# zjykzj/YOLOv4

Hardware: AMD Instinct MI355X
Metric: images/sec fwd+bwd @608x608 bs=64 per GPU (YOLOv4 training step: forward + YOLOLoss + backward) (higher is better)
Workload: dtype f32

## Files before the change

yolov4_amd/csrc/common.h:

```cpp
#pragma once
#include <hip/hip_runtime.h>
#include <stdint.h>
#include "../../include/yolov4_amd.h"

typedef float f32x4 __attribute__((ext_vector_type(4)));
typedef float f32x16 __attribute__((ext_vector_type(16)));
typedef unsigned int u32x4 __attribute__((ext_vector_type(4)));

#define Y4_CHECK_LAUNCH()                                   \
    do {                                                    \
        if (hipGetLastError() != hipSuccess) return Y4_ERR_LAUNCH; \
    } while (0)

static inline hipStream_t y4_stream(void* s) { return reinterpret_cast<hipStream_t>(s); }

#include <atomic>
struct Y4DynLds {
    std::atomic<unsigned long long> done{0ull};
    bool ensure(const void* kernel, size_t bytes) {
        int d = 0;
        if (hipGetDevice(&d) != hipSuccess) return false;
        if (d >= 0 && d < 64 && ((done.load(std::memory_order_acquire) >> d) & 1ull)) return true;
        if (hipFuncSetAttribute(kernel, hipFuncAttributeMaxDynamicSharedMemorySize, (int)bytes) != hipSuccess) return false;
        if (d >= 0 && d < 64) done.fetch_or(1ull << d, std::memory_order_release);
        return true;
    }
};

__device__ __forceinline__ float y4_mish(float x) {
    const float n = __expf(fminf(x, 20.0f));
    const float w = n * (n + 2.0f);
    return x * (w * __frcp_rn(w + 2.0f));
}
__device__ __forceinline__ float y4_mish_grad(float x) {
    const float n = __expf(fminf(x, 20.0f));
    const float w = n * (n + 2.0f);
    const float rd = __frcp_rn(w + 2.0f);
    const float q = fmaf(n, n, n);
    return fmaf(4.0f * (x * q), rd, w) * rd;
}
__device__ __forceinline__ float y4_act(float x, int act) {
    switch (act) {
        case Y4_ACT_LEAKY: return x > 0.0f ? x : 0.1f * x;
        case Y4_ACT_MISH: return y4_mish(x);
        case Y4_ACT_RELU: return fmaxf(x, 0.0f);
        default: return x;
    }
}
__device__ __forceinline__ float y4_act_grad(float x, int act) {
    switch (act) {
        case Y4_ACT_LEAKY: return x > 0.0f ? 1.0f : 0.1f;
        case Y4_ACT_MISH: return y4_mish_grad(x);
        case Y4_ACT_RELU: return x > 0.0f ? 1.0f : 0.0f;
        default: return 1.0f;
    }
}

template <int ACT> __device__ __forceinline__ float y4_act_t(float x) {
// ... 26 lines not shown
```

yolov4_amd/csrc/conv_planes.hip:

```cpp
#include <stdlib.h>
#include <type_traits>
#include "common.h"
#include "conv_geom.h"

namespace {

typedef _Float16 f16x8 __attribute__((ext_vector_type(8)));
typedef float f32x4v __attribute__((ext_vector_type(4)));

__device__ __host__ __forceinline__ unsigned pl_scale_exp(unsigned amax_bits) {
    const unsigned e = (amax_bits >> 23) & 0xffu;
    if (e == 0u || e == 255u) return 127u;
    int se = 268 - (int)e;
    if (se < 2) se = 2;
    if (se > 252) se = 252;
    return (unsigned)se;
}
__device__ __forceinline__ float pl_scale(const unsigned* amax) { return __uint_as_float(pl_scale_exp(amax ? *amax : 0u) << 23); }
__device__ __forceinline__ float pl_unscale(const unsigned* amax) { return __uint_as_float((254u - pl_scale_exp(amax ? *amax : 0u)) << 23); }

struct PlaneConvGeom {
    const unsigned char* src;
    const unsigned char* wt;
    float* dst; long long ldd;
    const float* res; long long ldr;
    float* stats;
    int dst_bf16;
    int cls_ntaps, cls_ph, cls_pw, Hfull, Wfull;
    int cls_dh[4], cls_dw[4], cls_slot[4];
    int B, Hs, Ws, Cs, Hd, Wd, N, k, stride, pad, M, K;
    int mtiles, ntiles;
    unsigned long long src_total_bytes;
    unsigned wt_bytes;
    const unsigned* src_amax; const unsigned* wt_amax;
};

constexpr int PROW = 128;

typedef __bf16 bf16x8 __attribute__((ext_vector_type(8)));
template <bool BF>
__device__ __forceinline__ f32x4v pl_mma(const f16x8 a, const f16x8 b, const f32x4v c) {
    if constexpr (BF) return __builtin_amdgcn_mfma_f32_16x16x32_bf16(__builtin_bit_cast(bf16x8, a), __builtin_bit_cast(bf16x8, b), c, 0, 0, 0);
    else return __builtin_amdgcn_mfma_f32_16x16x32_f16(a, b, c, 0, 0, 0);
}

#ifndef PL_ST_POL
#define PL_ST_POL 2
#endif
template <int BM, int BN, int WM, int WN, bool BF, bool YB = false, bool DG2 = false>
__global__ __launch_bounds__(WM * WN * 64, WM * WN == 8 ? 1 : 2) void conv_planes_mfma(const PlaneConvGeom g) {
    constexpr int NWAVE = WM * WN, NTHR = NWAVE * 64;
    static_assert(NWAVE == 8 || NWAVE == 4, "8 or 4 waves");
    constexpr int WTM = BM / WM, WTN = BN / WN, TM = WTM / 16, TN = WTN / 16;
    constexpr int A_BYTES = BM * PROW, B_BYTES = BN * PROW, STAGE = A_BYTES + B_BYTES;
    constexpr int NSTAGE = (NWAVE == 8 && 3 * STAGE <= 160 * 1024) ? 3 : 2;
    constexpr int KSH = BF ? 6 : 5;
    constexpr unsigned WEB = BF ? 2u : 4u;
    constexpr int PA = BM / 8 / NWAVE, PB = BN / 8 / NWAVE, NDMA = PA + PB;
    static_assert(PA >= 1 && PB >= 1 && ((NSTAGE == 3 && NDMA == 6) || (NSTAGE == 2 && NDMA == 8)),
                  "the counted vmcnt below assumes 6 (three stages) or 8 (two stages) pieces per wave and K-tile");
    typedef float accv __attribute__((ext_vector_type(4)));
    extern __shared__ __attribute__((aligned(1024))) unsigned char smem[];

    const int tid = threadIdx.x, lane = tid & 63;
    const int wave = __builtin_amdgcn_readfirstlane(tid >> 6);
    const int wm = wave / WN, wn = wave % WN;
    const int lt = y4_xcd_remap(blockIdx.x, g.mtiles * g.ntiles);
    const int mt = lt / g.ntiles, nt = lt - mt * g.ntiles;
    const int n0 = nt * BN;
    const int CC = g.Cs >> KSH;
    const int KT = (DG2 ? g.cls_ntaps : g.k * g.k) * CC;

    const int pix_per_img = g.Hd * g.Wd;
    const int b_first = (int)(((long long)mt * BM) / pix_per_img);
    const unsigned pitch = (unsigned)g.Cs * 4u;
    const unsigned long long img_bytes = (unsigned long long)g.Hs * g.Ws * pitch;
    const unsigned long long skip = (unsigned long long)b_first * img_bytes;
    const unsigned long long left = g.src_total_bytes > skip ? g.src_total_bytes - skip : 0ull;
    const __amdgpu_buffer_rsrc_t src_rsrc = y4_make_rsrc(g.src + skip, (unsigned)(left < 0xfffffff0ull ? left : 0xfffffff0ull));
    const __amdgpu_buffer_rsrc_t wt_rsrc = y4_make_rsrc(g.wt, g.wt_bytes);
    const unsigned OOB = 0xffffffffu;

    const int lr = lane >> 3, pos = lane & 7;
    unsigned a_base[PA], a_valid[PA], a_voff[PA];
#pragma unroll
    for (int i = 0; i < PA; ++i) {
        const int row = (wave * PA + i) * 8 + lr;
        const int m = mt * BM + row;
        const bool ok = m < g.M;
        const int mm = ok ? m : 0;
        const int b = mm / pix_per_img;
        const int rem = mm - b * pix_per_img;
        const int hd = rem / g.Wd, wd = rem - hd * g.Wd;
        const int hc = DG2 ? hd : hd * g.stride - g.pad, wc = DG2 ? wd : wd * g.stride - g.pad;
        const int chunk = pos ^ ((row >> 1) & 7);
        a_base[i] = (unsigned)(((b - b_first) * g.Hs + hc) * g.Ws + wc) * pitch + (unsigned)chunk * 16u;
        unsigned v = 0u;
        if constexpr (DG2) {
            for (int t = 0; t < g.cls_ntaps; ++t)
                if (ok && hc + g.cls_dh[t] < g.Hs && wc + g.cls_dw[t] < g.Ws) v |= 1u << t;
        } else {
            for (int r = 0; r < g.k; ++r)
                for (int q = 0; q < g.k; ++q)
                    if (ok && (unsigned)(hc + r) < (unsigned)g.Hs && (unsigned)(wc + q) < (unsigned)g.Ws) v |= 1u << (r * g.k + q);
        }
        a_valid[i] = v;
    }
    unsigned b_off[PB];
#pragma unroll
    for (int j = 0; j < PB; ++j) {
        const int row = (wave * PB + j) * 8 + lr;
        const int chunk = pos ^ ((row >> 1) & 7);
        b_off[j] = (n0 + row) < g.N ? (unsigned)(n0 + row) * (unsigned)g.K * WEB + (unsigned)chunk * 16u : OOB;
    }
    int ld_tap = 0, ld_r = 0, ld_q = 0, ld_cc = 0;
    int ld_slot = DG2 ? g.cls_slot[0] : 0;
    auto tap_setup = [&]() {
        unsigned toff;
        if constexpr (DG2) {
            const int t = ld_tap < g.cls_ntaps ? ld_tap : 0;
            toff = (unsigned)(g.cls_dh[t] * g.Ws + g.cls_dw[t]) * pitch;
            ld_slot = g.cls_slot[t];
        } else {
            toff = (unsigned)(ld_r * g.Ws + ld_q) * pitch;
            ld_slot = ld_tap;
        }
#pragma unroll
        for (int i = 0; i < PA; ++i) a_voff[i] = ((a_valid[i] >> ld_tap) & 1u) ? a_base[i] + toff : OOB;
    };
    tap_setup();
    typedef __attribute__((address_space(3))) void* lds_ptr;
    auto issue = [&](int stage, auto P0, auto P1) {
        constexpr int p0 = decltype(P0)::value, p1 = decltype(P1)::value;
        unsigned char* st = smem + stage * STAGE;
        const unsigned soff_a = (unsigned)ld_cc * 128u;
        const unsigned soff_b = (unsigned)(ld_slot * CC + ld_cc) * 128u;
#pragma unroll
        for (int p = p0; p < p1; ++p) {
            if (p < PA)
                __builtin_amdgcn_raw_ptr_buffer_load_lds(src_rsrc, (lds_ptr)(st + (wave * PA + p) * 1024), 16, (int)a_voff[p], (int)soff_a, 0, 0);
            else
                __builtin_amdgcn_raw_ptr_buffer_load_lds(wt_rsrc, (lds_ptr)(st + A_BYTES + (wave * PB + (p - PA)) * 1024), 16,
                                                         (int)b_off[p - PA], (int)soff_b, 0, 0);
        }
        if constexpr (p1 == NDMA) {
            if (++ld_cc == CC) {
                ld_cc = 0; ++ld_tap;
                if (++ld_q == g.k) { ld_q = 0; ++ld_r; }
                tap_setup();
            }
        }
    };
    using I0 = std::integral_constant<int, 0>; using I2 = std::integral_constant<int, 2>; using I4 = std::integral_constant<int, 4>;
    using I6 = std::integral_constant<int, NDMA>;

    accv acc0[TM][TN], acc1[BF ? 1 : TM][BF ? 1 : TN];
#pragma unroll
    for (int i = 0; i < TM; ++i)
#pragma unroll
        for (int j = 0; j < TN; ++j)
#pragma unroll
            for (int e = 0; e < 4; ++e) {
                acc0[i][j][e] = 0.f;
                if constexpr (!BF) acc1[i][j][e] = 0.f;
            }

    const int fr = lane & 15, kq = lane >> 4;
    const int sw = (fr >> 1) & 7;
    const int a_hi = (wm * WTM + fr) * PROW + ((kq ^ sw) << 4), a_lo = (wm * WTM + fr) * PROW + (((4 + kq) ^ sw) << 4);
    const int b_hi = A_BYTES + (wn * WTN + fr) * PROW + ((kq ^ sw) << 4), b_lo = A_BYTES + (wn * WTN + fr) * PROW + (((4 + kq) ^ sw) << 4);

    bool pend = false;
    auto step = [&](auto SC, const int kt) {
        constexpr int S = decltype(SC)::value;
        const unsigned char* base = smem + S * STAGE;
        f16x8 fb[TN][2];
#pragma unroll
        for (int j = 0; j < TN; ++j) {
            fb[j][0] = *reinterpret_cast<const f16x8*>(base + b_hi + j * 16 * PROW);
            fb[j][1] = *reinterpret_cast<const f16x8*>(base + b_lo + j * 16 * PROW);
        }
        f16x8 fap[2][2];
        fap[0][0] = *reinterpret_cast<const f16x8*>(base + a_hi);
        fap[0][1] = *reinterpret_cast<const f16x8*>(base + a_lo);
#pragma unroll
        for (int i = 0; i < TM; ++i) {
            if (i + 1 < TM) {
                fap[(i + 1) & 1][0] = *reinterpret_cast<const f16x8*>(base + a_hi + (i + 1) * 16 * PROW);
                fap[(i + 1) & 1][1] = *reinterpret_cast<const f16x8*>(base + a_lo + (i + 1) * 16 * PROW);
            }
            const f16x8 fa0 = fap[i & 1][0], fa1 = fap[i & 1][1];
            if (i == TM - 1) {
                __builtin_amdgcn_sched_barrier(0);
                asm volatile("s_waitcnt lgkmcnt(0)" ::: "memory");
                if (kt + 1 < KT) {
                    if constexpr (NSTAGE == 3) {
                        if (kt + 2 < KT) asm volatile("s_waitcnt vmcnt(6)" ::: "memory");
                        else asm volatile("s_waitcnt vmcnt(0)" ::: "memory");
                        __builtin_amdgcn_s_barrier();
                        if (kt + 3 < KT) { issue(S, I0{}, I2{}); pend = true; }
                    } else {
                        asm volatile("s_waitcnt vmcnt(0)" ::: "memory");
                        __builtin_amdgcn_s_barrier();
                        if (kt + 2 < KT) issue(S, I0{}, I6{});
                    }
                }
            }
            if constexpr (BF) {
#pragma unroll
                for (int j = 0; j < TN; ++j) acc0[i][j] = pl_mma<true>(fa0, fb[j][0], acc0[i][j]);
#pragma unroll
                for (int j = 0; j < TN; ++j) acc0[i][j] = pl_mma<true>(fa1, fb[j][1], acc0[i][j]);
            } else {
#pragma unroll
                for (int j = 0; j < TN; ++j) {
                    acc1[i][j] = pl_mma<false>(fa1, fb[j][0], acc1[i][j]);
                    acc1[i][j] = pl_mma<false>(fa0, fb[j][1], acc1[i][j]);
                    acc0[i][j] = pl_mma<false>(fa0, fb[j][0], acc0[i][j]);
                }
            }
            if constexpr (NSTAGE == 3) {
                if (i == 0 && pend) issue((S + 2) % NSTAGE, I2{}, I4{});
                if (i == 1 && pend) { issue((S + 2) % NSTAGE, I4{}, I6{}); pend = false; }
            }
        }
    };
    static_assert(TM >= 3, "the DMA pieces are spread over the first three row tiles");

    for (int t = 0; t < NSTAGE && t < KT; ++t) issue(t, I0{}, I6{});
    if constexpr (NSTAGE == 3) {
        if (KT >= 3) asm volatile("s_waitcnt vmcnt(12)" ::: "memory");
        else if (KT == 2) asm volatile("s_waitcnt vmcnt(6)" ::: "memory");
        else asm volatile("s_waitcnt vmcnt(0)" ::: "memory");
    } else {
        if (KT >= 2) asm volatile("s_waitcnt vmcnt(8)" ::: "memory");
        else asm volatile("s_waitcnt vmcnt(0)" ::: "memory");
    }
    __builtin_amdgcn_s_barrier();
    if constexpr (NSTAGE == 3) {
        int kt = 0;
        for (; kt + 3 <= KT; kt += 3) {
            step(std::integral_constant<int, 0>{}, kt);
            step(std::integral_constant<int, 1>{}, kt + 1);
            step(std::integral_constant<int, 2>{}, kt + 2);
        }
        if (kt < KT) step(std::integral_constant<int, 0>{}, kt);
        if (kt + 1 < KT) step(std::integral_constant<int, 1>{}, kt + 1);
    } else {
        int kt = 0;
        for (; kt + 2 <= KT; kt += 2) {
            step(std::integral_constant<int, 0>{}, kt);
            step(std::integral_constant<int, 1>{}, kt + 1);
        }
        if (kt < KT) step(std::integral_constant<int, 0>{}, kt);
    }

    const float un = BF ? 1.0f : pl_unscale(g.src_amax) * pl_unscale(g.wt_amax);
    const float un1 = un * (1.0f / 2048.0f);
    auto result = [&](int i, int j, int e) -> float {
        if constexpr (BF) return acc0[i][j][e];
        else return acc0[i][j][e] * un + acc1[i][j][e] * un1;
    };
    {
        const unsigned drow = (unsigned)g.ldd * 4u, rrow = (unsigned)g.ldr * 4u;
        const long long row0 = (long long)mt * BM;
        const unsigned long long left = (unsigned long long)(g.M - row0);
        const unsigned long long dby = left * drow, rby = g.ldr ? left * rrow : (unsigned long long)g.N * 4ull;
        const __amdgpu_buffer_rsrc_t drs = y4_make_rsrc(reinterpret_cast<char*>(g.dst) + row0 * (long long)drow, (unsigned)(dby < 0xfffffff0ull ? dby : 0xfffffff0ull));
        const __amdgpu_buffer_rsrc_t rrs = y4_make_rsrc(g.res ? reinterpret_cast<const char*>(g.res) + row0 * (long long)rrow : nullptr,
                                                        g.res ? (unsigned)(rby < 0xfffffff0ull ? rby : 0xfffffff0ull) : 0u);
        int lane_e = lane;
        asm volatile("" : "+v"(lane_e));
        const int fr = lane_e & 15, kq = lane_e >> 4;
        const int colb = n0 + wn * WTN + fr;
        const bool allc = n0 + BN <= g.N;
        if constexpr (DG2) {
            const __amdgpu_buffer_rsrc_t xrs = y4_make_rsrc(g.dst, (unsigned)((unsigned long long)g.B * g.Hfull * g.Wfull * drow));
#pragma unroll
            for (int i = 0; i < TM; ++i) {
                const int m0 = mt * BM + wm * WTM + 16 * i + 4 * kq;
                int b = m0 / pix_per_img;
                const int rem = m0 - b * pix_per_img;
                int hc = rem / g.Wd, wc = rem - hc * g.Wd;
#pragma unroll
                for (int e = 0; e < 4; ++e) {
                    const bool rok = m0 + e < g.M;
                    const unsigned po = (unsigned)((b * g.Hfull + 2 * hc + g.cls_ph) * g.Wfull + 2 * wc + g.cls_pw) * drow + (unsigned)colb * 4u;
#pragma unroll
                    for (int j = 0; j < TN; ++j) {
                        const float v = result(i, j, e);
// ... 45 lines not shown
                        const bool cok = allc || colb + 16 * j < g.N;
                        __builtin_amdgcn_raw_buffer_store_b32(__builtin_bit_cast(unsigned, v), drs, (int)(cok ? dvo + 64u * j : 0xffffffffu), (int)(e * drow), PL_ST_POL);
                    }
            }
        }
        } else {
            float csum[TN], cssum[TN];
#pragma unroll
            for (int j = 0; j < TN; ++j) { csum[j] = 0.f; cssum[j] = 0.f; }
#pragma unroll
            for (int i = 0; i < TM; ++i) {
                const unsigned rl = (unsigned)(wm * WTM + 16 * i + 4 * kq);
                const unsigned dvo = rl * drow + (unsigned)colb * 2u;
#pragma unroll
                for (int e = 0; e < 4; ++e)
#pragma unroll
                    for (int j = 0; j < TN; ++j) {
                        const float v = result(i, j, e);
                        unsigned u = __builtin_bit_cast(unsigned, v);
                        u = (u + 0x7fffu + ((u >> 16) & 1u)) & 0xffff0000u;
                        const float vr = __builtin_bit_cast(float, u);
                        csum[j] += vr; cssum[j] += vr * vr;
                        const unsigned nb = (unsigned)__builtin_amdgcn_update_dpp(0, (int)u, 0xB1, 0xf, 0xf, true);
                        const bool cok = (allc || colb + 16 * j < g.N) && !(fr & 1);
                        __builtin_amdgcn_raw_buffer_store_b32((u >> 16) | nb, drs, (int)(cok ? dvo + 32u * j : 0xffffffffu), (int)(e * drow), PL_ST_POL);
                    }
                __builtin_amdgcn_sched_barrier(0);
            }
#pragma unroll
            for (int j = 0; j < TN; ++j) { acc0[0][j][0] = csum[j]; acc0[0][j][1] = cssum[j]; }
        }
    }
    if (g.stats) {
        __syncthreads();
        float* red = reinterpret_cast<float*>(smem);
#pragma unroll
        for (int j = 0; j < TN; ++j) {
            float cs = 0.f, css = 0.f;
            if constexpr (YB) {
                cs = acc0[0][j][0]; css = acc0[0][j][1];
            } else {
#pragma unroll
                for (int i = 0; i < TM; ++i)
#pragma unroll
                    for (int e = 0; e < 4; ++e) { const float v = acc0[i][j][e]; cs += v; css += v * v; }
            }
            cs += __shfl_xor(cs, 16, 64); css += __shfl_xor(css, 16, 64);
            cs += __shfl_xor(cs, 32, 64); css += __shfl_xor(css, 32, 64);
            if (kq == 0) {
                const int c = wn * WTN + j * 16 + fr;
                red[(wm * BN + c) * 2 + 0] = cs;
                red[(wm * BN + c) * 2 + 1] = css;
            }
        }
        __syncthreads();
        for (int c = tid; c < BN; c += NTHR) {
            float cs = 0.f, css = 0.f;
#pragma unroll
            for (int w = 0; w < WM; ++w) { cs += red[(w * BN + c) * 2]; css += red[(w * BN + c) * 2 + 1]; }
            const int n = n0 + c;
            if (n < g.N) {
                g.stats[((long long)mt * 2 + 0) * g.N + n] = cs;
                g.stats[((long long)mt * 2 + 1) * g.N + n] = css;
            }
        }
    }
}

struct PlaneWgradGeom {
    const unsigned char* x;
    const unsigned char* dy;
    float* out;
    int B, H, W, Cin, Cout, k, pad, M, J;
    int ldy_ch;
    int ntn, ntj, splits, steps_per_split;
    unsigned long long x_total_bytes, dy_total_bytes;
    const unsigned* x_amax; const unsigned* dy_amax;
};

typedef __fp16 trh4 __attribute__((__vector_size__(4 * sizeof(__fp16))));
__device__ __forceinline__ f16x8 tr_frag(const unsigned char* p) {
    typedef __attribute__((address_space(3))) trh4* lp;
    const trh4 a = __builtin_amdgcn_ds_read_tr16_b64_v4f16((lp)(p));
    const trh4 b = __builtin_amdgcn_ds_read_tr16_b64_v4f16((lp)(p + 4 * PROW));
    f16x8 r;
#pragma unroll
    for (int e = 0; e < 4; ++e) { r[e] = (_Float16)a[e]; r[4 + e] = (_Float16)b[e]; }
    return r;
}

template <int N> __device__ __forceinline__ void pl_wait_vm() {
    static_assert(N == 0 || N == 3 || N == 4 || N == 6 || N == 8 || N == 12, "add the literal");
    if constexpr (N == 0) asm volatile("s_waitcnt vmcnt(0)" ::: "memory");
    else if constexpr (N == 3) asm volatile("s_waitcnt vmcnt(3)" ::: "memory");
    else if constexpr (N == 4) asm volatile("s_waitcnt vmcnt(4)" ::: "memory");
    else if constexpr (N == 6) asm volatile("s_waitcnt vmcnt(6)" ::: "memory");
    else if constexpr (N == 8) asm volatile("s_waitcnt vmcnt(8)" ::: "memory");
    else asm volatile("s_waitcnt vmcnt(12)" ::: "memory");
}
// ... 448 lines not shown
        if (nt == 1) return launch_stream_bf16<4, 1, 4, YB>(g, st, nparts);
        if (nt == 2) return launch_stream_bf16<4, 2, 4, YB>(g, st, nparts);
        return launch_stream_bf16<4, 4, 4, YB>(g, st, nparts);
    }
    if (nt == 1) return launch_stream_bf16<8, 1, 4, YB>(g, st, nparts);
    if (nt == 2) return launch_stream_bf16<8, 2, 4, YB>(g, st, nparts);
    return launch_stream_bf16<8, 4, 4, YB>(g, st, nparts);
}

__global__ __launch_bounds__(256) void bf16_filter_kernel(const float* __restrict__ w, unsigned short* __restrict__ fwd,
                                                          unsigned short* __restrict__ tr, int Cout, int Cin, int kk, int mirror) {
    const long long n = (long long)Cout * kk * Cin;
    const long long i0 = blockIdx.x * (long long)blockDim.x + threadIdx.x, step = (long long)gridDim.x * blockDim.x;
    if (fwd)
        for (long long i = i0; i < n; i += step) fwd[i] = pl_bf16_bits(w[i]);
    if (tr)
        for (long long i = i0; i < n; i += step) {
            const int nn = (int)(i % Cout);
            const long long t = i / Cout;
            const int tp = (int)(t % kk);
            const int tap = mirror ? kk - 1 - tp : tp;
            const int c = (int)(t / kk);
            tr[i] = pl_bf16_bits(w[((long long)nn * kk + tap) * Cin + c]);
        }
}
int bf16_filter(const float* w, unsigned short* fwd, unsigned short* tr, int Cout, int Cin, int kk, bool mirror, hipStream_t st) {
    const long long n = (long long)Cout * kk * Cin;
    const int blocks = (int)((n + 255) / 256 > 2048 ? 2048 : (n + 255) / 256);
    hipLaunchKernelGGL(bf16_filter_kernel, dim3(blocks > 0 ? blocks : 1), dim3(256), 0, st, w, fwd, tr, Cout, Cin, kk, mirror ? 1 : 0);
    Y4_CHECK_LAUNCH();
    return Y4_OK;
}

template <int BM, int BN, int WM, int WN, bool BF, bool YB = false, bool DG2 = false>
int launch_conv_planes(const PlaneConvGeom& g0, hipStream_t st) {
    PlaneConvGeom g = g0;
    g.mtiles = (g.M + BM - 1) / BM;
    g.ntiles = (g.N + BN - 1) / BN;
    constexpr int NW = WM * WN;
    constexpr size_t stage = (size_t)(BM + BN) * PROW;
    constexpr size_t smem = ((NW == 8 && 3 * stage <= 160 * 1024) ? 3ull : 2ull) * stage;
    static_assert(NW == 8 || 2 * smem <= 160 * 1024, "two blocks per CU");
    static_assert(smem <= 160 * 1024, "LDS");
    auto kern = conv_planes_mfma<BM, BN, WM, WN, BF, YB, DG2>;
    static Y4DynLds lds_attr;
    if (!lds_attr.ensure(reinterpret_cast<const void*>(kern), smem)) return Y4_ERR_LAUNCH;
    y4::note_kernel("conv_planes_mfma<%d, %d, %d, %d, %s, %s, %s>", BM, BN, WM, WN, BF ? "true" : "false", YB ? "true" : "false",
                    DG2 ? "true" : "false");
    hipLaunchKernelGGL(kern, dim3(g.mtiles * g.ntiles), dim3(NW * 64), smem, st, g);
    Y4_CHECK_LAUNCH();
    return Y4_OK;
}

}

namespace y4 {

bool planes_conv_ok(int Cin, int Cout, int k, int stride) {
    return Cin > 0 && (Cin & 31) == 0 && Cout > 0 && (Cout & 3) == 0 && (k == 1 || k == 3) && (stride == 1 || stride == 2);
}

static bool conv_window_ok(int B, int Hs, int Ws, int Cs, int N, int k, int stride, bool bf) {
    const int pad = (k - 1) / 2;
    const long long Hd = (Hs + 2 * pad - k) / stride + 1, Wd = (Ws + 2 * pad - k) / stride + 1;
    if (Hd <= 0 || Wd <= 0 || (long long)B * Hd * Wd >= (1ll << 31)) return false;
    const unsigned long long img = (unsigned long long)Hs * Ws * (unsigned long long)Cs * 4ull;
    const unsigned long long wb = (unsigned long long)N * k * k * Cs * (bf ? 2ull : 4ull);
    const unsigned long long imgs_per_tile = 256ull / (unsigned long long)(Hd * Wd) + 2;
    return img * imgs_per_tile < 0xfffffff0ull && wb < 0xfffffff0ull;
}
static bool dgrad_s2_window_ok(int B, int H, int W, int Cin, int Cout, long long lddx) {
    if ((H & 1) || (W & 1)) return false;
    return conv_window_ok(B, H / 2, W / 2, Cout, Cin, 3, 1, false) &&
           (unsigned long long)B * H * W * (unsigned long long)lddx * 4ull < 0xfffffff0ull;
}
static bool wgrad_window_ok(int B, int H, int W, int Cin, int Cout, int k, int stride, bool bf) {
    const long long M = (long long)B * H * W;
    if (M >= (1ll << 31) - 65536) return false;
    if ((unsigned long long)Cout * k * k * Cin * 4ull >= 0xfffffff0ull) return false;
    int ntn, ntj, splits, sps;
    planes_wgrad_plan(B, H, W, Cin, Cout, k, &ntn, &ntj, &splits, &sps, planes_wgrad_tn(Cout, bf), bf);
    const int pad = (k - 1) / 2;
// ... 34 lines not shown
    g.wt_bytes = (unsigned)wb;
    g.src_amax = src_amax; g.wt_amax = wt_amax;
    static const int small_mode = getenv("Y4_PLANES_SMALL") ? atoi(getenv("Y4_PLANES_SMALL")) : 1;
    bool quant = false;
    {
        const long long nt = (N + 127) / 128;
        const long long b256 = (long long)((g.M + 255) / 256) * nt, b128 = (long long)((g.M + 127) / 128) * nt;
        const long long c256 = ((b256 + 255) / 256) * 2;
        const long long tail = b128 % 512;
        const long long c128 = (b128 / 512) * 2 + (tail == 0 ? 0 : (tail <= 256 ? 1 : 2));
        quant = (double)c128 * 1.08 < (double)c256;
    }
    const bool small = small_mode == 2 || (small_mode == 1 && (g.K <= 256 || quant)) || (small_mode == 4 && g.K <= 256);
    if (bf && stream_bf16_ok(g, dst_bf16)) {
        g.K = Cs;
        return dst_bf16 ? dispatch_stream_bf16<true>(g, st, nparts) : dispatch_stream_bf16<false>(g, st, nparts);
    }
    if (bf) {
        const char* bt = getenv("Y4_BF_TILE");
        const int bf_tile = bt ? atoi(bt) : 0;
        const long long mt = (g.M + 255) / 256;
        const long long r256 = (mt * ((N + 255) / 256) + 255) / 256, r128 = (mt * ((N + 127) / 128) + 255) / 256;
        const bool big = bf_tile == 2 || (bf_tile == 0 && N > 128 && (double)r256 * 2.0 <= (double)r128 * 1.25);
        if (small && !big) {
            if (nparts) *nparts = (g.M + 127) / 128;
            return dst_bf16 ? launch_conv_planes<128, 128, 2, 2, true, true>(g, st) : launch_conv_planes<128, 128, 2, 2, true>(g, st);
        }
        if (nparts) *nparts = (g.M + 255) / 256;
        if (dst_bf16) return big ? launch_conv_planes<256, 256, 2, 4, true, true>(g, st) : launch_conv_planes<256, 128, 4, 2, true, true>(g, st);
        return big ? launch_conv_planes<256, 256, 2, 4, true>(g, st) : launch_conv_planes<256, 128, 4, 2, true>(g, st);
    }
    if (dst_bf16) return Y4_ERR_SHAPE;
    if (nparts) *nparts = small ? (g.M + 127) / 128 : (g.M + 255) / 256;
    return small ? launch_conv_planes<128, 128, 2, 2, false>(g, st) : launch_conv_planes<256, 128, 4, 2, false>(g, st);
}

int planes_dgrad_s2(const void* dy, const unsigned* dy_amax, const void* wt_planes, const unsigned* wt_amax, float* dx, long long lddx,
                    int B, int H, int W, int Cin, int Cout, hipStream_t st, bool bf) {
    if ((H & 1) || (W & 1) || (Cout & 31) || (Cin & 3) || (bf && (Cout & 63))) return Y4_ERR_SHAPE;
    const int Ho = H / 2, Wo = W / 2;
    PlaneConvGeom g{};
    g.src = static_cast<const unsigned char*>(dy); g.wt = static_cast<const unsigned char*>(wt_planes);
    g.dst = dx; g.ldd = lddx;
    g.B = B; g.Hs = Ho; g.Ws = Wo; g.Cs = Cout; g.N = Cin; g.k = 3; g.stride = 1; g.pad = 0;
    g.Hd = Ho; g.Wd = Wo; g.Hfull = H; g.Wfull = W;
    if (B <= 0 || Ho <= 0 || Wo <= 0 || !dgrad_s2_window_ok(B, H, W, Cin, Cout, lddx)) return Y4_ERR_SHAPE;
    const long long M = (long long)B * Ho * Wo;
    g.M = (int)M; g.K = 9 * Cout;
    const unsigned long long img = (unsigned long long)Ho * Wo * (unsigned long long)Cout * 4ull;
    const unsigned long long wb = (unsigned long long)Cin * g.K * (bf ? 2ull : 4ull);
    g.src_total_bytes = (unsigned long long)B * img;
    g.wt_bytes = (unsigned)wb;
    g.src_amax = dy_amax; g.wt_amax = wt_amax;
    for (int c = 3; c >= 0; --c) {
        const int ph = c >> 1, pw = c & 1;
        g.cls_ph = ph; g.cls_pw = pw; g.cls_ntaps = 0;
        for (int r = 0; r < 3; ++r)
            for (int q = 0; q < 3; ++q) {
                if (((ph + 1 - r) & 1) || ((pw + 1 - q) & 1)) continue;
                const int t = g.cls_ntaps++;
                g.cls_dh[t] = (ph + 1 - r) / 2; g.cls_dw[t] = (pw + 1 - q) / 2; g.cls_slot[t] = r * 3 + q;
            }
        const int rc = bf ? launch_conv_planes<256, 128, 4, 2, true, false, true>(g, st)
                          : launch_conv_planes<256, 128, 4, 2, false, false, true>(g, st);
        if (rc != Y4_OK) return rc;
    }
    return Y4_OK;
// ... 247 lines not shown
```

Baseline: 449.8.

## Make f32 planes conv kernel persistent with cross-tile DMA prefetch

Adds a persistent variant of the f32 planes MFMA conv kernel. The grid is capped at resident blocks (CU count times blocks per CU), and each block loops over output tiles. Per-tile row and filter offset tables are built in LDS and double-buffered, so the global-load pipeline can run straight into the next tile's K loop without draining. The aim is to remove the pipeline fill and drain at each tile and the wave-quantization tail. In exchange it adds LDS table reads in tap setup, extra barriers, and more LDS use, which could lower occupancy or stall. It is on by default through an environment variable.

```diff
diff --git a/yolov4_amd/csrc/common.h b/yolov4_amd/csrc/common.h
--- a/yolov4_amd/csrc/common.h
+++ b/yolov4_amd/csrc/common.h
@@ -24,6 +24,20 @@
         if (hipFuncSetAttribute(kernel, hipFuncAttributeMaxDynamicSharedMemorySize, (int)bytes) != hipSuccess) return false;
         if (d >= 0 && d < 64) done.fetch_or(1ull << d, std::memory_order_release);
         return true;
+    }
+};
+
+struct Y4CuCount {
+    std::atomic<int> n[64];
+    Y4CuCount() { for (auto& v : n) v.store(0, std::memory_order_relaxed); }
+    int get() {
+        int d = 0;
+        if (hipGetDevice(&d) != hipSuccess) return -1;
+        if (d >= 0 && d < 64) { const int c = n[d].load(std::memory_order_acquire); if (c > 0) return c; }
+        int c = 0;
+        if (hipDeviceGetAttribute(&c, hipDeviceAttributeMultiprocessorCount, d) != hipSuccess || c <= 0) return -1;
+        if (d >= 0 && d < 64) n[d].store(c, std::memory_order_release);
+        return c;
     }
 };
 
diff --git a/yolov4_amd/csrc/conv_planes.hip b/yolov4_amd/csrc/conv_planes.hip
--- a/yolov4_amd/csrc/conv_planes.hip
+++ b/yolov4_amd/csrc/conv_planes.hip
@@ -47,13 +47,40 @@
 #ifndef PL_ST_POL
 #define PL_ST_POL 2
 #endif
-template <int BM, int BN, int WM, int WN, bool BF, bool YB = false, bool DG2 = false>
-__global__ __launch_bounds__(WM * WN * 64, WM * WN == 8 ? 1 : 2) void conv_planes_mfma(const PlaneConvGeom g) {
+
+typedef unsigned long long pl_u64;
+__device__ __forceinline__ unsigned pl_lds_addr(const unsigned char* p) {
+    return (unsigned)(__UINTPTR_TYPE__)(__attribute__((address_space(3))) const unsigned char*)p;
+}
+__device__ __forceinline__ void pl_lds_st64(unsigned addr, unsigned lo, unsigned hi) {
+    const pl_u64 v = (pl_u64)lo | ((pl_u64)hi << 32);
+    asm volatile("ds_write_b64 %0, %1" ::"v"(addr), "v"(v) : "memory");
+}
+__device__ __forceinline__ void pl_lds_st32(unsigned addr, unsigned v) { asm volatile("ds_write_b32 %0, %1" ::"v"(addr), "v"(v) : "memory"); }
+__device__ __forceinline__ void pl_lds_ld64x4(unsigned addr, pl_u64 (&e)[4]) {
+    asm volatile("ds_read_b64 %0, %4\n\tds_read_b64 %1, %4 offset:64\n\tds_read_b64 %2, %4 offset:128\n\tds_read_b64 %3, %4 offset:192\n\t"
+                 "s_waitcnt lgkmcnt(0)"
+                 : "=&v"(e[0]), "=&v"(e[1]), "=&v"(e[2]), "=&v"(e[3]) : "v"(addr) : "memory");
+}
+template <int N> __device__ __forceinline__ void pl_lds_ld_hdr_rows(unsigned haddr, unsigned raddr, pl_u64& h0, unsigned& h1, unsigned (&r)[N]) {
+    static_assert(N == 2 || N == 4, "filter pieces per wave");
+    if constexpr (N == 2)
+        asm volatile("ds_read_b64 %0, %4\n\tds_read_b32 %1, %4 offset:8\n\tds_read_b32 %2, %5\n\tds_read_b32 %3, %5 offset:32\n\t"
+                     "s_waitcnt lgkmcnt(0)"
+                     : "=&v"(h0), "=&v"(h1), "=&v"(r[0]), "=&v"(r[1]) : "v"(haddr), "v"(raddr) : "memory");
+    else
+        asm volatile("ds_read_b64 %0, %6\n\tds_read_b32 %1, %6 offset:8\n\tds_read_b32 %2, %7\n\tds_read_b32 %3, %7 offset:32\n\t"
+                     "ds_read_b32 %4, %7 offset:64\n\tds_read_b32 %5, %7 offset:96\n\ts_waitcnt lgkmcnt(0)"
+                     : "=&v"(h0), "=&v"(h1), "=&v"(r[0]), "=&v"(r[1]), "=&v"(r[2]), "=&v"(r[3]) : "v"(haddr), "v"(raddr) : "memory");
+}
+template <int BM, int BN, int WM, int WN, bool BF, bool YB, bool DG2, bool PERSIST>
+__device__ __forceinline__ void conv_planes_body(const PlaneConvGeom& g) {
     constexpr int NWAVE = WM * WN, NTHR = NWAVE * 64;
     static_assert(NWAVE == 8 || NWAVE == 4, "8 or 4 waves");
     constexpr int WTM = BM / WM, WTN = BN / WN, TM = WTM / 16, TN = WTN / 16;
     constexpr int A_BYTES = BM * PROW, B_BYTES = BN * PROW, STAGE = A_BYTES + B_BYTES;
     constexpr int NSTAGE = (NWAVE == 8 && 3 * STAGE <= 160 * 1024) ? 3 : 2;
+    constexpr int RED_BYTES = WM * BN * 2 * 4;
     constexpr int KSH = BF ? 6 : 5;
     constexpr unsigned WEB = BF ? 2u : 4u;
     constexpr int PA = BM / 8 / NWAVE, PB = BN / 8 / NWAVE, NDMA = PA + PB;
@@ -65,27 +92,27 @@
     const int tid = threadIdx.x, lane = tid & 63;
     const int wave = __builtin_amdgcn_readfirstlane(tid >> 6);
     const int wm = wave / WN, wn = wave % WN;
-    const int lt = y4_xcd_remap(blockIdx.x, g.mtiles * g.ntiles);
-    const int mt = lt / g.ntiles, nt = lt - mt * g.ntiles;
-    const int n0 = nt * BN;
+    const int ntot = g.mtiles * g.ntiles;
+    const int G = PERSIST ? (int)gridDim.x : ntot;
+    const int NTAP = DG2 ? g.cls_ntaps : g.k * g.k;
     const int CC = g.Cs >> KSH;
-    const int KT = (DG2 ? g.cls_ntaps : g.k * g.k) * CC;
+    const int KT = NTAP * CC;
 
     const int pix_per_img = g.Hd * g.Wd;
-    const int b_first = (int)(((long long)mt * BM) / pix_per_img);
     const unsigned pitch = (unsigned)g.Cs * 4u;
     const unsigned long long img_bytes = (unsigned long long)g.Hs * g.Ws * pitch;
-    const unsigned long long skip = (unsigned long long)b_first * img_bytes;
-    const unsigned long long left = g.src_total_bytes > skip ? g.src_total_bytes - skip : 0ull;
-    const __amdgpu_buffer_rsrc_t src_rsrc = y4_make_rsrc(g.src + skip, (unsigned)(left < 0xfffffff0ull ? left : 0xfffffff0ull));
     const __amdgpu_buffer_rsrc_t wt_rsrc = y4_make_rsrc(g.wt, g.wt_bytes);
     const unsigned OOB = 0xffffffffu;
 
-    const int lr = lane >> 3, pos = lane & 7;
-    unsigned a_base[PA], a_valid[PA], a_voff[PA];
-#pragma unroll
-    for (int i = 0; i < PA; ++i) {
-        const int row = (wave * PA + i) * 8 + lr;
+    auto tile_origin = [&](const int ltile, int& mt, int& n0, int& b_first, unsigned long long& skip, unsigned& bytes) __attribute__((always_inline)) {
+        const int lt = y4_xcd_remap(ltile, ntot);
+        mt = lt / g.ntiles; n0 = (lt - mt * g.ntiles) * BN;
+        b_first = (int)(((long long)mt * BM) / pix_per_img);
+        skip = (unsigned long long)b_first * img_bytes;
+        const unsigned long long left = g.src_total_bytes > skip ? g.src_total_bytes - skip : 0ull;
+        bytes = (unsigned)(left < 0xfffffff0ull ? left : 0xfffffff0ull);
+    };
+    auto row_state = [&](const int mt, const int b_first, const int row, unsigned& base, unsigned& valid) __attribute__((always_inline)) {
         const int m = mt * BM + row;
         const bool ok = m < g.M;
         const int mm = ok ? m : 0;
@@ -93,8 +120,7 @@
         const int rem = mm - b * pix_per_img;
         const int hd = rem / g.Wd, wd = rem - hd * g.Wd;
         const int hc = DG2 ? hd : hd * g.stride - g.pad, wc = DG2 ? wd : wd * g.stride - g.pad;
-        const int chunk = pos ^ ((row >> 1) & 7);
-        a_base[i] = (unsigned)(((b - b_first) * g.Hs + hc) * g.Ws + wc) * pitch + (unsigned)chunk * 16u;
+        base = (unsigned)(((b - b_first) * g.Hs + hc) * g.Ws + wc) * pitch;
         unsigned v = 0u;
         if constexpr (DG2) {
             for (int t = 0; t < g.cls_ntaps; ++t)
@@ -104,18 +130,76 @@
                 for (int q = 0; q < g.k; ++q)
                     if (ok && (unsigned)(hc + r) < (unsigned)g.Hs && (unsigned)(wc + q) < (unsigned)g.Ws) v |= 1u << (r * g.k + q);
         }
-        a_valid[i] = v;
-    }
-    unsigned b_off[PB];
-#pragma unroll
-    for (int j = 0; j < PB; ++j) {
-        const int row = (wave * PB + j) * 8 + lr;
-        const int chunk = pos ^ ((row >> 1) & 7);
-        b_off[j] = (n0 + row) < g.N ? (unsigned)(n0 + row) * (unsigned)g.K * WEB + (unsigned)chunk * 16u : OOB;
+        valid = v;
+    };
+    auto filter_row = [&](const int n0, const int row) -> unsigned { return (n0 + row) < g.N ? (unsigned)(n0 + row) * (unsigned)g.K * WEB : OOB; };
+    constexpr int TAB_B = BM * 8, TAB_H = TAB_B + BN * 4, TAB_BYTES = TAB_H + 16;
+    constexpr int TAB0 = NSTAGE * STAGE + 2 * RED_BYTES;
+    static_assert(NTHR >= BM && NTHR >= BN, "one table row per thread");
+    auto table_fill = [&](const int ltile, const int buf) __attribute__((always_inline)) {
+        int mt, n0, b_first; unsigned long long skip; unsigned bytes;
+        tile_origin(ltile, mt, n0, b_first, skip, bytes);
+        const unsigned tab = pl_lds_addr(smem + TAB0 + buf * TAB_BYTES);
+        int t = tid;
+        asm volatile("" : "+v"(t));
+        if (t < BM) {
+            unsigned base, valid;
+            row_state(mt, b_first, t, base, valid);
+            pl_lds_st64(tab + t * 8, base, valid);
+        }
+        if (t < BN) pl_lds_st32(tab + TAB_B + t * 4, filter_row(n0, t));
+        if (t == 0) {
+            pl_lds_st64(tab + TAB_H, (unsigned)skip, (unsigned)(skip >> 32));
+            pl_lds_st32(tab + TAB_H + 8, bytes);
+        }
+    };
+    __amdgpu_buffer_rsrc_t src_rsrc;
+    unsigned a_base[PERSIST ? 1 : PA], a_valid[PERSIST ? 1 : PA], a_voff[PA], b_off[PB];
+    int ld_lt = blockIdx.x;
+    int ld_buf = 0;
+    auto table_read = [&]() __attribute__((always_inline)) {
+        const unsigned tab = pl_lds_addr(smem + TAB0 + ld_buf * TAB_BYTES);
+        int lane_s = lane;
+        asm volatile("" : "+v"(lane_s));
+        const int lr = lane_s >> 3, pos = lane_s & 7;
+        pl_u64 sk; unsigned by, o[PB];
+        pl_lds_ld_hdr_rows<PB>(tab + TAB_H, tab + TAB_B + (wave * PB * 8 + lr) * 4, sk, by, o);
+        const unsigned long long skip = (unsigned long long)(unsigned)__builtin_amdgcn_readfirstlane((int)(unsigned)sk) |
+                                        ((unsigned long long)(unsigned)__builtin_amdgcn_readfirstlane((int)(unsigned)(sk >> 32)) << 32);
+        src_rsrc = y4_make_rsrc(g.src + skip, (unsigned)__builtin_amdgcn_readfirstlane((int)by));
+#pragma unroll
+        for (int j = 0; j < PB; ++j) {
+            const int row = (wave * PB + j) * 8 + lr;
+            const int chunk = pos ^ ((row >> 1) & 7);
+            b_off[j] = o[j] != OOB ? o[j] + (unsigned)chunk * 16u : OOB;
+        }
+    };
+    if constexpr (PERSIST) {
+        table_fill(ld_lt, 0);
+        asm volatile("s_waitcnt lgkmcnt(0)" ::: "memory");
+        __builtin_amdgcn_s_barrier();
+        table_read();
+    } else {
+        int mt, n0, b_first; unsigned long long skip; unsigned bytes;
+        tile_origin(ld_lt, mt, n0, b_first, skip, bytes);
+        src_rsrc = y4_make_rsrc(g.src + skip, bytes);
+        const int lr = lane >> 3, pos = lane & 7;
+#pragma unroll
+        for (int i = 0; i < PA; ++i) {
+            const int row = (wave * PA + i) * 8 + lr;
+            row_state(mt, b_first, row, a_base[i], a_valid[i]);
+            a_base[i] += (unsigned)(pos ^ ((row >> 1) & 7)) * 16u;
+        }
+#pragma unroll
+        for (int j = 0; j < PB; ++j) {
+            const int row = (wave * PB + j) * 8 + lr;
+            const unsigned o = filter_row(n0, row);
+            b_off[j] = o != OOB ? o + (unsigned)(pos ^ ((row >> 1) & 7)) * 16u : OOB;
+        }
     }
     int ld_tap = 0, ld_r = 0, ld_q = 0, ld_cc = 0;
     int ld_slot = DG2 ? g.cls_slot[0] : 0;
-    auto tap_setup = [&]() {
+    auto tap_setup = [&]() __attribute__((always_inline)) {
         unsigned toff;
         if constexpr (DG2) {
             const int t = ld_tap < g.cls_ntaps ? ld_tap : 0;
@@ -125,14 +209,29 @@
             toff = (unsigned)(ld_r * g.Ws + ld_q) * pitch;
             ld_slot = ld_tap;
         }
-#pragma unroll
-        for (int i = 0; i < PA; ++i) a_voff[i] = ((a_valid[i] >> ld_tap) & 1u) ? a_base[i] + toff : OOB;
+        if constexpr (PERSIST) {
+            static_assert(!PERSIST || PA == 4, "pl_lds_ld64x4");
+            int lane_s = lane;
+            asm volatile("" : "+v"(lane_s));
+            const int lr = lane_s >> 3, pos = lane_s & 7;
+            pl_u64 e[4];
+            pl_lds_ld64x4(pl_lds_addr(smem + TAB0 + ld_buf * TAB_BYTES) + (wave * PA * 8 + lr) * 8, e);
+#pragma unroll
+            for (int i = 0; i < PA; ++i) {
+                const int row = (wave * PA + i) * 8 + lr;
+                const int chunk = pos ^ ((row >> 1) & 7);
+                a_voff[i] = (((unsigned)(e[i] >> 32) >> ld_tap) & 1u) ? (unsigned)e[i] + (unsigned)chunk * 16u + toff : OOB;
+            }
+        } else {
+#pragma unroll
+            for (int i = 0; i < PA; ++i) a_voff[i] = ((a_valid[i] >> ld_tap) & 1u) ? a_base[i] + toff : OOB;
+        }
     };
     tap_setup();
     typedef __attribute__((address_space(3))) void* lds_ptr;
-    auto issue = [&](int stage, auto P0, auto P1) {
+    auto issue = [&](const int soff, auto P0, auto P1, auto PRO) __attribute__((always_inline)) {
         constexpr int p0 = decltype(P0)::value, p1 = decltype(P1)::value;
-        unsigned char* st = smem + stage * STAGE;
+        unsigned char* st = smem + soff;
         const unsigned soff_a = (unsigned)ld_cc * 128u;
         const unsigned soff_b = (unsigned)(ld_slot * CC + ld_cc) * 128u;
 #pragma unroll
@@ -147,23 +246,31 @@
             if (++ld_cc == CC) {
                 ld_cc = 0; ++ld_tap;
                 if (++ld_q == g.k) { ld_q = 0; ++ld_r; }
+                if constexpr (PERSIST) {
+                    if (ld_tap == NTAP) {
+                        ld_tap = 0; ld_r = 0; ld_q = 0;
+                        ld_lt += G; ld_buf ^= 1;
+                        if (ld_lt < ntot) {
+                            if constexpr (decltype(PRO)::value) {
+                                asm volatile("s_waitcnt lgkmcnt(0)" ::: "memory");
+                                __builtin_amdgcn_s_barrier();
+                                table_fill(ld_lt, ld_buf);
+                                asm volatile("s_waitcnt lgkmcnt(0)" ::: "memory");
+                                __builtin_amdgcn_s_barrier();
+                            }
+                            table_read();
+                        }
+                    }
+                }
                 tap_setup();
             }
         }
     };
+    using LOOP = std::false_type; using PROLOGUE = std::true_type;
     using I0 = std::integral_constant<int, 0>; using I2 = std::integral_constant<int, 2>; using I4 = std::integral_constant<int, 4>;
     using I6 = std::integral_constant<int, NDMA>;
 
     accv acc0[TM][TN], acc1[BF ? 1 : TM][BF ? 1 : TN];
-#pragma unroll
-    for (int i = 0; i < TM; ++i)
-#pragma unroll
-        for (int j = 0; j < TN; ++j)
-#pragma unroll
-            for (int e = 0; e < 4; ++e) {
-                acc0[i][j][e] = 0.f;
-                if constexpr (!BF) acc1[i][j][e] = 0.f;
-            }
 
     const int fr = lane & 15, kq = lane >> 4;
     const int sw = (fr >> 1) & 7;
@@ -171,9 +278,12 @@
     const int b_hi = A_BYTES + (wn * WTN + fr) * PROW + ((kq ^ sw) << 4), b_lo = A_BYTES + (wn * WTN + fr) * PROW + (((4 + kq) ^ sw) << 4);
 
     bool pend = false;
-    auto step = [&](auto SC, const int kt) {
-        constexpr int S = decltype(SC)::value;
-        const unsigned char* base = smem + S * STAGE;
+    int pend_off = 0;
+    auto step = [&](auto SO, auto SO2, const int ahead, const bool drain) __attribute__((always_inline)) {
+        int so = SO;
+        const int so2 = SO2;
+        if constexpr (PERSIST) asm volatile("" : "+s"(so));
+        const unsigned char* base = smem + so;
         f16x8 fb[TN][2];
 #pragma unroll
         for (int j = 0; j < TN; ++j) {
@@ -193,16 +303,16 @@
             if (i == TM - 1) {
                 __builtin_amdgcn_sched_barrier(0);
                 asm volatile("s_waitcnt lgkmcnt(0)" ::: "memory");
-                if (kt + 1 < KT) {
+                if (ahead >= 1) {
                     if constexpr (NSTAGE == 3) {
-                        if (kt + 2 < KT) asm volatile("s_waitcnt vmcnt(6)" ::: "memory");
+                        if (ahead >= 2 && !drain) asm volatile("s_waitcnt vmcnt(6)" ::: "memory");
                         else asm volatile("s_waitcnt vmcnt(0)" ::: "memory");
                         __builtin_amdgcn_s_barrier();
-                        if (kt + 3 < KT) { issue(S, I0{}, I2{}); pend = true; }
+                        if (ahead >= 3) { issue(so, I0{}, I2{}, LOOP{}); pend = true; pend_off = so; }
                     } else {
                         asm volatile("s_waitcnt vmcnt(0)" ::: "memory");
                         __builtin_amdgcn_s_barrier();
-                        if (kt + 2 < KT) issue(S, I0{}, I6{});
+                        if (ahead >= 2) issue(so, I0{}, I6{}, LOOP{});
                     }
                 }
             }
@@ -220,42 +330,95 @@
                 }
             }
             if constexpr (NSTAGE == 3) {
-                if (i == 0 && pend) issue((S + 2) % NSTAGE, I2{}, I4{});
-                if (i == 1 && pend) { issue((S + 2) % NSTAGE, I4{}, I6{}); pend = false; }
+                if (i == 0 && pend) issue(so2, I2{}, I4{}, LOOP{});
+                if (i == 1 && pend) { issue(so2, I4{}, I6{}, LOOP{}); pend = false; }
             }
         }
     };
     static_assert(TM >= 3, "the DMA pieces are spread over the first three row tiles");
 
-    for (int t = 0; t < NSTAGE && t < KT; ++t) issue(t, I0{}, I6{});
+    float un_blk = 1.0f;
+    if constexpr (PERSIST && !BF)
+        un_blk = __builtin_bit_cast(float, __builtin_amdgcn_readfirstlane(__builtin_bit_cast(int, pl_unscale(g.src_amax) * pl_unscale(g.wt_amax))));
+
+    const int my_tiles = PERSIST ? (ntot - (int)blockIdx.x + G - 1) / G : 1;
+    int ahead = my_tiles * KT - 1;
+    for (int t = 0; t < NSTAGE && t <= ahead; ++t) issue(t * STAGE, I0{}, I6{}, PROLOGUE{});
     if constexpr (NSTAGE == 3) {
-        if (KT >= 3) asm volatile("s_waitcnt vmcnt(12)" ::: "memory");
-        else if (KT == 2) asm volatile("s_waitcnt vmcnt(6)" ::: "memory");
+        if (ahead >= 2) asm volatile("s_waitcnt vmcnt(12)" ::: "memory");
+        else if (ahead == 1) asm volatile("s_waitcnt vmcnt(6)" ::: "memory");
         else asm volatile("s_waitcnt vmcnt(0)" ::: "memory");
     } else {
-        if (KT >= 2) asm volatile("s_waitcnt vmcnt(8)" ::: "memory");
+        if (ahead >= 1) asm volatile("s_waitcnt vmcnt(8)" ::: "memory");
         else asm volatile("s_waitcnt vmcnt(0)" ::: "memory");
     }
     __builtin_amdgcn_s_barrier();
-    if constexpr (NSTAGE == 3) {
-        int kt = 0;
-        for (; kt + 3 <= KT; kt += 3) {
-            step(std::integral_constant<int, 0>{}, kt);
-            step(std::integral_constant<int, 1>{}, kt + 1);
-            step(std::integral_constant<int, 2>{}, kt + 2);
-        }
-        if (kt < KT) step(std::integral_constant<int, 0>{}, kt);
-        if (kt + 1 < KT) step(std::integral_constant<int, 1>{}, kt + 1);
+
+    int rot = 0;
+    int par = 0;
+    for (int ct = blockIdx.x;;) {
+    const int lt = y4_xcd_remap(ct, ntot);
+    const int mt = lt / g.ntiles, nt = lt - mt * g.ntiles;
+    const int n0 = nt * BN;
+    const bool first = ct == (int)blockIdx.x;
+    if constexpr (PERSIST) {
+        if (ld_lt + G < ntot) table_fill(ld_lt + G, ld_buf ^ 1);
+    }
+#pragma unroll
+    for (int i = 0; i < TM; ++i)
+#pragma unroll
+        for (int j = 0; j < TN; ++j)
+#pragma unroll
+            for (int e = 0; e < 4; ++e) {
+                acc0[i][j][e] = 0.f;
+                if constexpr (!BF) acc1[i][j][e] = 0.f;
+            }
+    if constexpr (!PERSIST) {
+        using S0 = std::integral_constant<int, 0>; using S1 = std::integral_constant<int, STAGE>; using S2 = std::integral_constant<int, 2 * STAGE>;
+        if constexpr (NSTAGE == 3) {
+            int kt = 0;
+            for (; kt + 3 <= KT; kt += 3) {
+                step(S0{}, S2{}, KT - 1 - kt, false);
+                step(S1{}, S0{}, KT - 2 - kt, false);
+                step(S2{}, S1{}, KT - 3 - kt, false);
+            }
+            if (kt < KT) step(S0{}, S2{}, KT - 1 - kt, false);
+            if (kt + 1 < KT) step(S1{}, S0{}, KT - 2 - kt, false);
+        } else {
+            int kt = 0;
+            for (; kt + 2 <= KT; kt += 2) {
+                step(S0{}, S0{}, KT - 1 - kt, false);
+                step(S1{}, S1{}, KT - 2 - kt, false);
+            }
+            if (kt < KT) step(S0{}, S0{}, KT - 1 - kt, false);
+        }
     } else {
-        int kt = 0;
-        for (; kt + 2 <= KT; kt += 2) {
-            step(std::integral_constant<int, 0>{}, kt);
-            step(std::integral_constant<int, 1>{}, kt + 1);
-        }
-        if (kt < KT) step(std::integral_constant<int, 0>{}, kt);
-    }
-
-    const float un = BF ? 1.0f : pl_unscale(g.src_amax) * pl_unscale(g.wt_amax);
+        const int o0 = rot * STAGE, o1 = (rot + 1 == NSTAGE ? 0 : rot + 1) * STAGE;
+        if constexpr (NSTAGE == 3) {
+            const int o2 = (rot == 0 ? 2 : rot - 1) * STAGE;
+            int kt = 0;
+            for (; kt + 3 <= KT; kt += 3) {
+                step(o0, o2, ahead, kt == 0 && !first);
+                step(o1, o0, ahead - 1, false);
+                step(o2, o1, ahead - 2, false);
+                ahead -= 3;
+            }
+            if (kt < KT) { step(o0, o2, ahead, kt == 0 && !first); --ahead; }
+            if (kt + 1 < KT) { step(o1, o0, ahead, false); --ahead; }
+            if (pend) { issue(pend_off, I2{}, I6{}, LOOP{}); pend = false; }
+        } else {
+            int kt = 0;
+            for (; kt + 2 <= KT; kt += 2) {
+                step(o0, o0, ahead, false);
+                step(o1, o1, ahead - 1, false);
+                ahead -= 2;
+            }
+            if (kt < KT) { step(o0, o0, ahead, false); --ahead; }
+        }
+        rot = (rot + KT) % NSTAGE;
+    }
+
+    const float un = PERSIST ? un_blk : BF ? 1.0f : pl_unscale(g.src_amax) * pl_unscale(g.wt_amax);
     const float un1 = un * (1.0f / 2048.0f);
     auto result = [&](int i, int j, int e) -> float {
         if constexpr (BF) return acc0[i][j][e];
@@ -367,8 +530,8 @@
         }
     }
     if (g.stats) {
-        __syncthreads();
-        float* red = reinterpret_cast<float*>(smem);
+        if constexpr (!PERSIST) __syncthreads();
+        float* red = reinterpret_cast<float*>(smem + (PERSIST ? NSTAGE * STAGE + par * RED_BYTES : 0));
 #pragma unroll
         for (int j = 0; j < TN; ++j) {
             float cs = 0.f, css = 0.f;
@@ -388,7 +551,12 @@
                 red[(wm * BN + c) * 2 + 1] = css;
             }
         }
-        __syncthreads();
+        if constexpr (PERSIST) {
+            asm volatile("s_waitcnt lgkmcnt(0)" ::: "memory");
+            __builtin_amdgcn_s_barrier();
+        } else {
+            __syncthreads();
+        }
         for (int c = tid; c < BN; c += NTHR) {
             float cs = 0.f, css = 0.f;
 #pragma unroll
@@ -400,6 +568,22 @@
             }
         }
     }
+    if constexpr (!PERSIST) break;
+    else {
+        ct += G;
+        if (ct >= ntot) break;
+        par ^= 1;
+    }
+    }
+}
+
+template <int BM, int BN, int WM, int WN, bool BF, bool YB = false, bool DG2 = false>
+__global__ __launch_bounds__(WM * WN * 64, WM * WN == 8 ? 1 : 2) void conv_planes_mfma(const PlaneConvGeom g) {
+    conv_planes_body<BM, BN, WM, WN, BF, YB, DG2, false>(g);
+}
+template <int BM, int BN, int WM, int WN, bool BF, bool YB = false, bool DG2 = false>
+__global__ __launch_bounds__(WM * WN * 64, WM * WN == 8 ? 1 : 2) void conv_planes_mfma_persist(const PlaneConvGeom g) {
+    conv_planes_body<BM, BN, WM, WN, BF, YB, DG2, true>(g);
 }
 
 struct PlaneWgradGeom {
@@ -914,22 +1098,35 @@
     return Y4_OK;
 }
 
-template <int BM, int BN, int WM, int WN, bool BF, bool YB = false, bool DG2 = false>
-int launch_conv_planes(const PlaneConvGeom& g0, hipStream_t st) {
+template <int BM, int BN, int WM, int WN, bool BF, bool YB = false, bool DG2 = false, bool PERSIST = false>
+int launch_conv_planes(const PlaneConvGeom& g0, hipStream_t st, int cap = 0) {
     PlaneConvGeom g = g0;
     g.mtiles = (g.M + BM - 1) / BM;
     g.ntiles = (g.N + BN - 1) / BN;
     constexpr int NW = WM * WN;
     constexpr size_t stage = (size_t)(BM + BN) * PROW;
-    constexpr size_t smem = ((NW == 8 && 3 * stage <= 160 * 1024) ? 3ull : 2ull) * stage;
+    constexpr size_t smem = ((NW == 8 && 3 * stage <= 160 * 1024) ? 3ull : 2ull) * stage + (PERSIST ? 2ull * (WM * BN * 8 + BM * 8 + BN * 4 + 16) : 0ull);
     static_assert(NW == 8 || 2 * smem <= 160 * 1024, "two blocks per CU");
     static_assert(smem <= 160 * 1024, "LDS");
-    auto kern = conv_planes_mfma<BM, BN, WM, WN, BF, YB, DG2>;
+    void (*kern)(const PlaneConvGeom);
+    if constexpr (PERSIST) kern = conv_planes_mfma_persist<BM, BN, WM, WN, BF, YB, DG2>;
+    else kern = conv_planes_mfma<BM, BN, WM, WN, BF, YB, DG2>;
     static Y4DynLds lds_attr;
     if (!lds_attr.ensure(reinterpret_cast<const void*>(kern), smem)) return Y4_ERR_LAUNCH;
-    y4::note_kernel("conv_planes_mfma<%d, %d, %d, %d, %s, %s, %s>", BM, BN, WM, WN, BF ? "true" : "false", YB ? "true" : "false",
-                    DG2 ? "true" : "false");
-    hipLaunchKernelGGL(kern, dim3(g.mtiles * g.ntiles), dim3(NW * 64), smem, st, g);
+    int blocks = g.mtiles * g.ntiles;
+    if constexpr (PERSIST) {
+        static Y4CuCount cus;
+        const int resident = cus.get() * (NW == 8 ? 1 : 2);
+        if (resident <= 0) return Y4_ERR_LAUNCH;
+        const int most = cap > 0 ? cap : resident;
+        if (blocks > most) blocks = most;
+        y4::note_kernel("conv_planes_mfma_persist<%d, %d, %d, %d, %s, %s, %s>", BM, BN, WM, WN, BF ? "true" : "false", YB ? "true" : "false",
+                        DG2 ? "true" : "false");
+    } else {
+        y4::note_kernel("conv_planes_mfma<%d, %d, %d, %d, %s, %s, %s>", BM, BN, WM, WN, BF ? "true" : "false", YB ? "true" : "false",
+                        DG2 ? "true" : "false");
+    }
+    hipLaunchKernelGGL(kern, dim3(blocks), dim3(NW * 64), smem, st, g);
     Y4_CHECK_LAUNCH();
     return Y4_OK;
 }
@@ -1030,7 +1227,12 @@
     }
     if (dst_bf16) return Y4_ERR_SHAPE;
     if (nparts) *nparts = small ? (g.M + 127) / 128 : (g.M + 255) / 256;
-    return small ? launch_conv_planes<128, 128, 2, 2, false>(g, st) : launch_conv_planes<256, 128, 4, 2, false>(g, st);
+    const char* pe = getenv("Y4_PLANES_PERSIST");
+    const int persist = pe ? atoi(pe) : 1;
+    if (persist <= 0) return small ? launch_conv_planes<128, 128, 2, 2, false>(g, st) : launch_conv_planes<256, 128, 4, 2, false>(g, st);
+    const int cap = persist >= 2 ? persist : 0;
+    return small ? launch_conv_planes<128, 128, 2, 2, false, false, false, true>(g, st, cap)
+                 : launch_conv_planes<256, 128, 4, 2, false, false, false, true>(g, st, cap);
 }
 
 int planes_dgrad_s2(const void* dy, const unsigned* dy_amax, const void* wt_planes, const unsigned* wt_amax, float* dx, long long lddx,
```

Result: no change. 452.8, median of 6 (+0.7%).
